# tusen-ai/simpledet

Measured on AMD Instinct MI355X. Metric: images/sec at 800x1333 FPN 512-RoI RoIAlign fwd+bwd, higher is better.
Workload: dtype f32; 1 GPU; fused FPN RoIAlign_v2 fwd+bwd, P2-P5 256ch 800x1333, N=2 img/GPU, 512 RoIs/img, 7x7x4 samples (BASELINE configs[1]); images_per_gpu=2, rois_per_image=512, argmax_state=packed u8 (decoded in backward)

## Files before the change

simpledet_amd/csrc/roi_align_common.h:

```cpp
#pragma once
#include "common.h"
#include "../../include/simpledet_ops.h"
#include <float.h>
#include <math.h>
#include <type_traits>
#include <hip/hip_fp16.h>

namespace sd {

struct RoiLevels {
  const float* data[SD_MAX_FPN_LEVELS];
  int H[SD_MAX_FPN_LEVELS], W[SD_MAX_FPN_LEVELS], stride[SD_MAX_FPN_LEVELS];
  float scale[SD_MAX_FPN_LEVELS];
  int nlvl;
  float canon_scale, canon_level, k_min, k_max;
};

__device__ __forceinline__ int fpn_level(float x1, float y1, float x2, float y2,
                                         const RoiLevels& L) {
  float area = (x2 - x1 + 1.f) * (y2 - y1 + 1.f);
  float s = sqrtf(area);
  float t = floorf(L.canon_level + log2f(s / L.canon_scale + 1e-6f));
  t = t < L.k_min ? L.k_min : (t > L.k_max ? L.k_max : t);
  if (!(t == t)) return -1;
// ... 162 lines not shown
constexpr int kBandHalo = 8;
constexpr int kBandMaxBands = 16;
constexpr int kBandNP = 4;
constexpr int kBandMaxUnits = 512;
constexpr int kBandFillCost = 140, kBandPlaneCost = 60, kBandSetupCost = 1500;
constexpr int kBandSub = 4;
constexpr int kBandFallbackWGs = 0;

typedef float v2f __attribute__((ext_vector_type(2)));

struct BandPlan {
  int owned[SD_MAX_FPN_LEVELS];
  int rows[SD_MAX_FPN_LEVELS];
  int nbands[SD_MAX_FPN_LEVELS];
  int g[SD_MAX_FPN_LEVELS];
  int unit_base[SD_MAX_FPN_LEVELS];
  int halo[SD_MAX_FPN_LEVELS];
  int nwg;
  int nunits;
  int grab;
  int gbias;
  int tail;
  int tail_planes;
  int pool;
  uint4* rowent;
  uint4* colent;
  float2* rowval;
  float2* colval;
  unsigned* items;
  int2* seg;
  unsigned char* fbflag;
  int* chan_ctr;
  int nlist, nent;
};

struct BandArgs {
  FwdArgs f;
  BandPlan p;
};

struct BwdArgs {
  RoiLevels L;
  const float* dy;
  const float* ax;
  const float* ay;
  const float* rois;
  float* dx;
  int B, C, R, PP, H, W;
  float scale;
  int filter_lvl;
  int band_rows, nbands;
  int req;
  int ablate;
};

struct BwdFusedArgs {
  RoiLevels L;
  const float* dy;
  const float* ax;
  const float* ay;
  const unsigned char* amax8;
  const float* coords;
  const float* rois;
  float* dx[SD_MAX_FPN_LEVELS];
  int band_rows[SD_MAX_FPN_LEVELS], nbands[SD_MAX_FPN_LEVELS];
  int block_end[SD_MAX_FPN_LEVELS];
// ... 33 lines not shown
```

simpledet_amd/csrc/roi_align_fwd.hip:

```cpp
#include "roi_align_common.h"

namespace sd {

__global__ __launch_bounds__(256) void roi_align_fwd_naive(FwdArgs a) {
  const int PP = a.PH * a.PW;
  const long count = (long)a.B * a.R * a.C * PP;
  for (long index = (long)blockIdx.x * blockDim.x + threadIdx.x; index < count;
       index += (long)gridDim.x * blockDim.x) {
    int pw = (int)(index % a.PW);
    int ph = (int)((index / a.PW) % a.PH);
    int c = (int)((index / PP) % a.C);
    int n = (int)(index / PP / a.C);
    const float* r = a.rois + (long)n * 4;
    float x1 = r[0], y1 = r[1], x2 = r[2], y2 = r[3];
    int lvl = 0;
    if (a.L.nlvl > 1) lvl = fpn_level(x1, y1, x2, y2, a.L);
    FwdOut o{0.f, -1.f, -1.f, 255};
    if (lvl >= 0) {
      int H = a.L.H[lvl], W = a.L.W[lvl];
      const float* plane = a.L.data[lvl] + ((long)(n / a.R) * a.C + c) * H * W;
      o = roi_align_fwd_elem(plane, H, W, x1, y1, x2, y2, a.L.scale[lvl], ph, pw, a.PH, a.PW);
    }
    if (a.L.nlvl > 1) o.val = o.val + 0.0f;
    a.out[index] = o.val;
    if (a.amax8) {
      a.amax8[((long)n * a.C + c) * amax_stride(PP) + ph * a.PW + pw] = (unsigned char)o.code;
    } else {
      a.ax[index] = o.ax;
      a.ay[index] = o.ay;
    }
  }
}

// ... 373 lines not shown
  }
}

template <int PH, int PW, int NROI, bool PK>
__global__ __launch_bounds__(512) void roi_align_fwd_tiled(FwdArgs a) {
  __shared__ FwdSmem<PH, PW, NROI> s;
  fwd_tiled_body<PH, PW, NROI, PK>(a, s, blockIdx.x);
}

__device__ __forceinline__ int band_fill(const float* gsrc, int len, float* buf, int wave, int lane) {
  const int shift = (int)(((uintptr_t)gsrc >> 2) & 3);
  const float* a0 = gsrc - shift;
  const int n4 = (shift + len + 3) >> 2;
  const int first_full = shift ? 1 : 0;
  const int last_full = ((shift + len) >> 2);
  const float4* s4 = reinterpret_cast<const float4*>(a0);
  float4* d4 = reinterpret_cast<float4*>(buf);
  for (int w4 = wave * kWave; w4 < last_full; w4 += kBandWaves * kWave) {
    const int i = w4 + lane;
    if (i >= first_full && i < last_full) __builtin_amdgcn_global_load_lds(s4 + i, d4 + w4, 16, 0, 0);
  }
  if (wave == 0) {
    if (shift && lane < 4 && lane >= shift && lane < shift + len)
      __builtin_amdgcn_global_load_lds(a0 + lane, buf, 4, 0, 0);
    if (last_full < n4 && last_full >= first_full && (last_full > 0 || !shift)) {
      const int j = last_full * 4 + lane;
      if (lane < 4 && j < shift + len) __builtin_amdgcn_global_load_lds(a0 + j, buf + last_full * 4, 4, 0, 0);
    }
  }
  return shift;
}

template <int POOL, bool PK, bool HALF = false>
__global__ __launch_bounds__(kBandThreads) void roi_align_fwd_band(BandArgs A) {
  using TIn = typename std::conditional<HALF, __half, float>::type;
  constexpr int AL = HALF ? 8 : 4;
  const FwdArgs& a = A.f;
  const BandPlan& P = A.p;
  constexpr int QL = POOL, IPP = kWave / QL;
  constexpr int NP = (PK && !HALF) ? kBandNP : kBandNP - 1, CAP = NP * kBandWaves * IPP;
  constexpr int PPG = POOL * POOL, PPSG = amax_stride(PPG);
  extern __shared__ __attribute__((aligned(16))) float band_smem[];
  const int tid = threadIdx.x, lane = tid & (kWave - 1);
  const int wave = __builtin_amdgcn_readfirstlane(tid / kWave);

#ifdef SD_PROFILING
  const long long t_entry = __builtin_readcyclecounter();
#endif
  __shared__ int v_unit[kBandMaxUnits], v_first[kBandMaxUnits], v_items[kBandMaxUnits];
  __shared__ int v_cost[kBandMaxUnits], v_start[kBandMaxUnits + 1];
  __shared__ int2 s_grab[2];
  __shared__ int s_pick;
  const int wg = (int)blockIdx.x - kBandFallbackWGs, nwg = (int)gridDim.x - kBandFallbackWGs;
  const int rsub = (a.R + kBandSub - 1) / kBandSub;
  auto level_of = [&](int u) {
    int l = 0;
    for (int k = 0; k < a.L.nlvl; ++k)
      if (a.L.stride[k] >= 0 && u >= P.unit_base[k]) l = k;
    return l;
  };
  __shared__ int s_nvu;
  auto wave_incl_scan = [&](int v) {
#pragma unroll
    for (int o = 1; o < kWave; o <<= 1) {
      const int t = __shfl_up(v, o);
      if (lane >= o) v += t;
    }
// ... 430 lines not shown
    for (int n0 = wg / nsl; n0 < nroi && wg / nsl < nslots; n0 += nslots * kWave) {
      const int nl = n0 + lane * nslots;
      int myflag = nl < nroi ? P.fbflag[nl] : 0;
      if (fast_void && myflag == 2) myflag = 0;
      unsigned long long todo = __ballot(myflag != 0);
      while (todo) {
      const int src = __builtin_ctzll(todo);
      todo &= todo - 1;
      const int n = n0 + src * nslots;
      const int flag = __builtin_amdgcn_readlane(myflag, src);
      const float4 bx = *reinterpret_cast<const float4*>(a.rois + (long)n * 4);
      const int lvl = a.L.nlvl > 1 ? fpn_level(bx.x, bx.y, bx.z, bx.w, a.L) : 0;
      for (int e = tid; e < csl * PPG; e += kBandThreads) {
        const int c = slice * csl + e / PPG, g = e % PPG;
        FwdOut o{0.f, -1.f, -1.f, 255};
        if (lvl >= 0 && flag == 1) {
          const int H = a.L.H[lvl], W = a.L.W[lvl];
          o = roi_align_fwd_elem(reinterpret_cast<const TIn*>(a.L.data[lvl]) + ((long)(n / a.R) * a.C + c) * H * W,
                                 H, W, bx.x, bx.y, bx.z, bx.w, a.L.scale[lvl], g / POOL, g % POOL, POOL, POOL);
        }
        if (a.L.nlvl > 1) o.val = o.val + 0.0f;
        if constexpr (HALF) reinterpret_cast<__half*>(a.out)[((long)n * a.C + c) * PPG + g] = __float2half(o.val);
        else a.out[((long)n * a.C + c) * PPG + g] = o.val;
        if (PK) {
          a.amax8[((long)n * a.C + c) * PPSG + g] = (unsigned char)o.code;
        } else {
          a.ax[((long)n * a.C + c) * PPG + g] = o.ax;
          a.ay[((long)n * a.C + c) * PPG + g] = o.ay;
        }
      }
      }
    }
    }
#ifdef SD_PROFILING
  if (a.dbg && lane == 0) {
    long long* d = a.dbg + ((long)blockIdx.x * kBandWaves + wave) * 8;
    d[0] = t_setup; d[1] = t_wait; d[2] = t_comp; d[3] = dbg_count;
    d[4] = __builtin_readcyclecounter() - t_begin; d[5] = t_begin - t_entry; d[6] = dbg_units; d[7] = t_begin;
  }
#endif
}

__global__ __launch_bounds__(512) void roi_align_fwd_quad(BandArgs A) {
  extern __shared__ __attribute__((aligned(16))) float band_smem[];
  const FwdArgs& a = A.f;
  const BandPlan& P = A.p;
  constexpr int T = 512, POOL = 7, PPG = POOL * POOL, NW = T / kWave;
  const int tid = threadIdx.x, lane = tid & (kWave - 1);
  const int wave = __builtin_amdgcn_readfirstlane(tid / kWave);
  const int G = a.C / 4;
  const int c = 4 * ((G & 7) == 0 ? (int)(blockIdx.x & 7) * (G >> 3) + (int)(blockIdx.x >> 3) : (int)blockIdx.x);
  const int img = blockIdx.y;
  const int H = a.L.H[0], W = a.L.W[0], HW = H * W;
  float4* pl = reinterpret_cast<float4*>(band_smem);
  float* st = band_smem + 4 * (HW + 1) + wave * (4 * PPG);
  const float* src = reinterpret_cast<const float*>(a.L.data[0]) + ((long)img * a.C + c) * HW;
  if ((HW & 3) == 0) {
    for (int i4 = tid; i4 < (HW >> 2); i4 += T) {
      const float4 v0 = *reinterpret_cast<const float4*>(src + 4 * i4);
      const float4 v1 = *reinterpret_cast<const float4*>(src + (long)HW + 4 * i4);
      const float4 v2 = *reinterpret_cast<const float4*>(src + 2L * HW + 4 * i4);
      const float4 v3 = *reinterpret_cast<const float4*>(src + 3L * HW + 4 * i4);
      pl[4 * i4 + 0] = make_float4(v0.x, v1.x, v2.x, v3.x);
      pl[4 * i4 + 1] = make_float4(v0.y, v1.y, v2.y, v3.y);
      pl[4 * i4 + 2] = make_float4(v0.z, v1.z, v2.z, v3.z);
      pl[4 * i4 + 3] = make_float4(v0.w, v1.w, v2.w, v3.w);
// ... 188 lines not shown
      int nbn = H <= rb ? 1 : (H + (rb - halo) - 1) / (rb - halo);
      const int cap = kBandNP * kBandWaves * (kWave / POOL);
      const long est = (long)a.R * POOL / (nvalid_lv > 0 ? nvalid_lv : 1);
      const int by_items = (int)((est * 5 + 4L * cap - 1) / (4L * cap));
      if (by_items > nbn && a.amax8) nbn = by_items;
      if (nbn > H) nbn = H;
      if (nbn > kBandMaxBands) nbn = kBandMaxBands;
      int owned = (H + nbn - 1) / nbn;
      if (nbn > 1)
        for (int o = owned; o < owned + 4 && o + halo <= rb; ++o)
          if (((long)o * W) % 4 == 0) { owned = o; break; }
      if (owned + halo > rb) owned = rb - halo;
      nbn = (H + owned - 1) / owned;
      if (nbn > kBandMaxBands) { ok = false; break; }
      P.nbands[l] = nbn;
      P.halo[l] = halo;
      P.owned[l] = nbn == 1 ? H : owned;
      P.rows[l] = nbn == 1 ? H : (owned + halo < H ? owned + halo : H);
      const long bstride = a.half_io ? (((long)P.rows[l] * W + 14) >> 3) * 8 : (((long)P.rows[l] * W + 4 + 3) & ~3L);
      int g = 1;
      for (int c = 2; c <= 8 && c <= gmax; c *= 2)
        if (a.C % c == 0 && c * bstride <= kBandBufFloats) g = c;
      if (bstride > kBandBufFloats) { ok = false; break; }
      P.g[l] = g;
      P.unit_base[l] = units;
      units += a.B * P.nbands[l];
    }
    auto al16 = [](size_t x) { return (x + 15) & ~(size_t)15; };
    const size_t ent = al16((size_t)nroi * POOL * sizeof(uint4));
    const size_t valb = a.amax8 ? 0 : al16((size_t)nroi * POOL * sizeof(float2));
    const size_t itemb = al16((size_t)a.B * SD_MAX_FPN_LEVELS * kBandSub * ((a.R + kBandSub - 1) / kBandSub) *
                              POOL * sizeof(unsigned));
    const size_t segb = al16((size_t)units * kBandSub * sizeof(int2));
    const size_t need = 16 + 2 * ent + 2 * valb + itemb + segb + al16(nroi) + kBandMaxUnits * sizeof(int);
    int wg = 0;
    P.nunits = units;
    P.grab = 4;
    P.gbias = 0;
    P.tail = 0;
    P.tail_planes = 8;
    {
      const int np = (a.amax8 && !a.half_io) ? kBandNP : kBandNP - 1;
      const long cap_launch = (long)np * kBandWaves * (kWave / POOL);
      if (units + (long)nroi * POOL / cap_launch > kBandMaxUnits) ok = false;
    }
    wg = kNumCU;
    if (ok && need <= workspace_bytes) {
      char* w = reinterpret_cast<char*>(((uintptr_t)workspace + 15) & ~(uintptr_t)15);
      P.rowent = reinterpret_cast<uint4*>(w); w += ent;
      P.colent = reinterpret_cast<uint4*>(w); w += ent;
      if (valb) {
        P.rowval = reinterpret_cast<float2*>(w); w += valb;
        P.colval = reinterpret_cast<float2*>(w); w += valb;
      }
      P.items = reinterpret_cast<unsigned*>(w); w += itemb;
      P.seg = reinterpret_cast<int2*>(w); w += segb;
      P.fbflag = reinterpret_cast<unsigned char*>(w); w += al16(nroi);
      P.chan_ctr = reinterpret_cast<int*>(w);
      P.nwg = wg;
      P.pool = POOL;
      A.f = a;
      const int nlist = a.B * a.L.nlvl * kBandSub, nent = cdiv((long)nroi * 2 * POOL, kBandThreads);
      const int ncoord = a.amax8 ? cdiv((long)nroi * 6 * POOL, kBandThreads) : 0;
      P.nlist = nlist; P.nent = nent;
      const int smem = 2 * kBandBufFloats * (int)sizeof(float);
      const bool merged = bplan && bplan->lists_units > 0 && bplan->PP == POOL * POOL;
      if (bplan_done) *bplan_done = merged;
      if (int e = launch_fwd_prep(A, POOL, nlist + nent + ncoord, merged ? bplan : nullptr, st)) return e;
      {
        const long HW0 = (long)a.L.H[0] * a.L.W[0];
        const size_t lds = (size_t)(HW0 + 1) * 16 + 8 * 4 * 49 * sizeof(float);
        if (!a.amax8 && !a.half_io && POOL == 7 && a.L.nlvl == 1 && a.L.stride[0] >= 0 && P.nbands[0] == 1 &&
            a.C % 4 == 0 && lds <= 78 * 1024 && a.B <= 65535 &&
            (((uintptr_t)a.L.data[0] | (uintptr_t)a.out | (uintptr_t)a.ax | (uintptr_t)a.ay) & 15) == 0 &&
            tuning("roi_align_fwd_quad", 1) == 1) {
          SD_HIP_CHECK(hipFuncSetAttribute((const void*)roi_align_fwd_quad, hipFuncAttributeMaxDynamicSharedMemorySize, (int)lds));
          hipLaunchKernelGGL(roi_align_fwd_quad, dim3(a.C / 4, a.B), dim3(512), lds, st, A);
          note_dispatch("sd::roi_fwd_prep_kernel<7> + sd::roi_align_fwd_quad");
          SD_LAUNCH_CHECK();
          return SD_OK;
        }
      }
#define SD_FWD_BAND(POOLV, PK)                                                                    \
  do {                                                                                            \
    auto k = roi_align_fwd_band<POOLV, PK>;                                                       \
    SD_HIP_CHECK(hipFuncSetAttribute((const void*)k, hipFuncAttributeMaxDynamicSharedMemorySize,  \
                                     smem));                                                      \
    hipLaunchKernelGGL(k, dim3(wg + kBandFallbackWGs), dim3(kBandThreads), smem, st, A);          \
  } while (0)
      if (a.half_io) {
#define SD_FWD_BAND_H(POOLV)                                                                      \
  do {                                                                                            \
    auto k = roi_align_fwd_band<POOLV, true, true>;                                               \
    SD_HIP_CHECK(hipFuncSetAttribute((const void*)k, hipFuncAttributeMaxDynamicSharedMemorySize,  \
                                     smem));                                                      \
    hipLaunchKernelGGL(k, dim3(wg + kBandFallbackWGs), dim3(kBandThreads), smem, st, A);          \
  } while (0)
        if (POOL == 7) SD_FWD_BAND_H(7); else SD_FWD_BAND_H(14);
#undef SD_FWD_BAND_H
      } else if (POOL == 7) {
        if (a.amax8) SD_FWD_BAND(7, true); else SD_FWD_BAND(7, false);
      } else {
        if (a.amax8) SD_FWD_BAND(14, true); else SD_FWD_BAND(14, false);
      }
#undef SD_FWD_BAND
      note_dispatch("sd::%s<%d> + sd::roi_align_fwd_band<%d,%s,%s>", merged ? "roi_prep_merged_kernel" : "roi_fwd_prep_kernel",
                    POOL, POOL, a.amax8 ? "true" : "false", a.half_io ? "true" : "false");
      SD_LAUNCH_CHECK();
      return SD_OK;
    }
  }
  if (a.half_io)
    return fail(SD_ERR_UNSUPPORTED, "fp16 RoIAlign runs on the band-resident kernel only: it needs the workspace, "
                "7x7 or 14x14 pooling, W in [2, 4095] and roi_align_fwd = 1, roi_align_fwd_band = 1");
  note_dispatch("sd::roi_align_fwd (tiled / naive fallback kernels: no workspace or a shape the band kernel does not take)");
  if (variant >= 1 && wide && a.PH == 7 && a.PW == 7) {
    if (a.amax8)
      hipLaunchKernelGGL((roi_align_fwd_tiled<7, 7, 4, true>), dim3(cdiv(nroi, 4) * a.nslice), dim3(512), 0, st, a);
    else
      hipLaunchKernelGGL((roi_align_fwd_tiled<7, 7, 4, false>), dim3(cdiv(nroi, 4) * a.nslice), dim3(512), 0, st, a);
  } else if (variant >= 1 && wide && a.PH == 14 && a.PW == 14) {
    if (a.amax8)
      hipLaunchKernelGGL((roi_align_fwd_tiled<14, 14, 1, true>), dim3(nroi * a.nslice), dim3(512), 0,
                         st, a);
    else
      hipLaunchKernelGGL((roi_align_fwd_tiled<14, 14, 1, false>), dim3(nroi * a.nslice), dim3(512),
                         0, st, a);
  } else {
    const int grid = (int)((count + 255) / 256 < 65536 * 16 ? (count + 255) / 256 : 65536 * 16);
    hipLaunchKernelGGL(roi_align_fwd_naive, dim3(grid), dim3(256), 0, st, a);
    if (a.amax8)
      hipLaunchKernelGGL(roi_coords_kernel, dim3(nroi), dim3(64), 0, st, a.rois, nroi, a.L, a.PH,
                         a.PW, a.coords);
  }
  SD_LAUNCH_CHECK();
  return SD_OK;
}

int check_dims(int B, int C, int R, int ph, int pw) {
  SD_REQUIRE(B >= 0 && C >= 0 && R >= 0, "negative dimension (B=%d C=%d R=%d)", B, C, R);
// ... 184 lines not shown
```

simpledet_amd/csrc/roi_align_lists.h:

```cpp
#pragma once
#include "roi_align_common.h"

namespace sd {

template <int PH, int PW, int THREADS>
__device__ __forceinline__ void bwd_band_list(const BwdFusedArgs& a, int lvl, int img, int nbands, int row0,
                                              int row1, float4 rb0, int* list, int* nlist, int* wcnt) {
  constexpr int NW = THREADS / kWave;
  const int tid = threadIdx.x, wave = tid / kWave, lane = tid & (kWave - 1);
  const int H = a.L.H[lvl];
  const float scale = a.L.scale[lvl];
  int base = 0, bound_sum = 0;
  for (int r0 = 0; r0 < a.R; r0 += THREADS) {
    const int r = r0 + tid;
    bool take = r < a.R && !(SD_ABLATE(a, 4));
    int weight = 0;
    if (take) {
      const float4 rb = r0 == 0 ? rb0 : *reinterpret_cast<const float4*>(a.rois + ((long)img * a.R + r) * 4);
      if (a.filter) take = fpn_level(rb.x, rb.y, rb.z, rb.w, a.L) == lvl;
      if (take && nbands > 1) {
        float s = fminr(fmaxr(rb.y * scale, 0.f), (float)(H - 1));
        float e = fminr(fmaxr(rb.w * scale, 0.f), (float)(H - 1));
        float lo = fminr(s, e) - 2.f, hi = fmaxr(s, e) + 2.f;
        if (hi < (float)row0 || lo > (float)(row1 - 1)) take = false;
      }
      if (take) {
        const float bwx = (rb.z - rb.x) * scale * (1.f / (float)PW), bwy = (rb.w - rb.y) * scale * (1.f / (float)PH);
        const float fx = 2.00002f * __builtin_amdgcn_rcpf(bwx), fy = 2.00002f * __builtin_amdgcn_rcpf(bwy);
        const int nx = (bwx > 0.f && fx < (float)PW) ? iminr((int)fx + 2, PW) : PW;
        const int ny = (bwy > 0.f && fy < (float)PH) ? iminr((int)fy + 2, PH) : PH;
        weight = nx * ny;
      }
    }
    const unsigned long long mask = __ballot(take);
    bound_sum += wave_sum_i32(weight);
    if (r0 > 0) __syncthreads();
    if (lane == 0) wcnt[wave] = __popcll(mask);
    __syncthreads();
    int off = base, total = 0;
#pragma unroll
    for (int w = 0; w < NW; ++w) {
      const int n = wcnt[w];
      if (w < wave) off += n;
      total += n;
    }
    if (take) list[off + __popcll(mask & ((1ull << lane) - 1))] = r;
    base += total;
  }
  if (lane == 0) atomicAdd(nlist + 1, bound_sum);
  if (tid == 0) nlist[0] = base;
  __syncthreads();
}

}
```

simpledet_amd/csrc/roi_align_prep.hip:

```cpp
#include "roi_align_lists.h"

namespace sd {

template <int POOL>
__device__ __forceinline__ void band_prep_block(const BandArgs& A, const int pblock, int nlist, int nent) {
  const FwdArgs& a = A.f;
  const BandPlan& P = A.p;
  const int tid = threadIdx.x, lane = tid & (kWave - 1);
  constexpr int LPR = POOL <= 8 ? 8 : 16;
  constexpr int RPP = kBandThreads / LPR;
  if (pblock < nlist) {
    __shared__ int hist[kBandMaxBands], cursor[kBandMaxBands];
    const int sub = pblock % kBandSub, lvl = (pblock / kBandSub) % a.L.nlvl;
    const int img = pblock / (kBandSub * a.L.nlvl);
    if (a.L.stride[lvl] < 0) return;
    int first_valid = 0;
    while (a.L.stride[first_valid] < 0) ++first_valid;
    const int H = a.L.H[lvl], W = a.L.W[lvl], nb = P.nbands[lvl], owned = P.owned[lvl];
    const float scale = a.L.scale[lvl];
    const int rsub = (a.R + kBandSub - 1) / kBandSub;
    const int rbeg = sub * rsub, rend = rbeg + rsub < a.R ? rbeg + rsub : a.R;
    if (tid < kBandMaxBands) hist[tid] = 0;
    __syncthreads();
    const int rr = tid / LPR, p = tid % LPR;
// ... 55 lines not shown
      int run = 0;
      for (int b = 0; b < nb; ++b) {
        cursor[b] = run;
        P.seg[(P.unit_base[lvl] + img * nb + b) * kBandSub + sub] = make_int2(run, hist[b]);
        run += hist[b];
      }
    }
    __syncthreads();
    auto emit = [&](int n, int band) {
      unsigned long long todo = __ballot(band >= 0);
      while (todo) {
        const int src = __builtin_ctzll(todo);
        const int bb = __builtin_amdgcn_readlane(band, src);
        const unsigned long long m = __ballot(band == bb);
        int base = 0;
        if (lane == src) base = atomicAdd(&cursor[bb], __popcll(m));
        base = __builtin_amdgcn_readlane(base, src);
        if (band == bb)
          items[base + __builtin_amdgcn_mbcnt_hi((unsigned)(m >> 32), __builtin_amdgcn_mbcnt_lo((unsigned)m, 0))] =
              (unsigned)n | ((unsigned)p << 16);
        todo &= ~m;
      }
    };
#pragma unroll
    for (int k = 0; k < KP; ++k)
      if (k < npass) emit(rbeg + k * RPP + rr, keep[k]);
    for (int k = KP; k < npass; ++k) {
      const int n = rbeg + k * RPP + rr;
      emit(n, classify(n));
    }
    return;
  }
  if (pblock == nlist && tid < kBandMaxUnits) P.chan_ctr[tid] = 0;
  const int eb = pblock - nlist;
  const int nroi = a.B * a.R;
  if (eb < nent) {
    const long e = (long)eb * kBandThreads + tid;
    if (e >= (long)nroi * 2 * POOL) return;
    const int p = (int)(e % POOL), ax = (int)((e / POOL) % 2), n = (int)(e / (2 * POOL));
    const float4 bx = *reinterpret_cast<const float4*>(a.rois + (long)n * 4);
    const int lvl = a.L.nlvl > 1 ? fpn_level(bx.x, bx.y, bx.z, bx.w, a.L) : 0;
    if (lvl < 0) return;
    const int H = a.L.H[lvl], W = a.L.W[lvl];
    float val[2] = {0.f, 0.f}, frac[2] = {0.f, 0.f};
    int off[4];
    const int cnt = ax == 0 ? axis_samples(p, POOL, bx.y, bx.w, a.L.scale[lvl], H, W, val, frac, off)
                            : axis_samples(p, POOL, bx.x, bx.z, a.L.scale[lvl], W, 1, val, frac, off);
    const float qnan = __int_as_float(0x7fc00000);
    const bool v0 = cnt >= 1, v1 = cnt >= 2;
    uint4 en;
    if (ax == 0) {
      en.x = (v0 ? (unsigned)off[0] | (off[1] != off[0] ? 1u << 20 : 0u) : 0u) | (cnt < 0 ? 1u << 31 : 0u);
      en.y = v1 ? (unsigned)off[2] | (off[3] != off[2] ? 1u << 20 : 0u) : 0u;
    } else {
      en.x = (v0 ? (unsigned)off[0] | (off[1] == off[0] ? 1u << 12 : 0u) : 0u) |
             (v1 ? (unsigned)off[2] << 13 | (off[3] == off[2] ? 1u << 25 : 0u) : 0u) | (cnt < 0 ? 1u << 26 : 0u);
      en.y = 0u;
    }
    en.z = __float_as_uint(v0 ? frac[0] : qnan);
    en.w = __float_as_uint(v1 ? frac[1] : qnan);
    (ax == 0 ? P.rowent : P.colent)[(long)n * POOL + p] = en;
    if (P.rowval) (ax == 0 ? P.rowval : P.colval)[(long)n * POOL + p] = make_float2(val[0], val[1]);
    return;
  }
  if (a.amax8) {
    const long e = (long)(eb - nent) * kBandThreads + tid;
    if (e >= (long)nroi * 6 * POOL) return;
    const int j = (int)(e % (6 * POOL)), n = (int)(e / (6 * POOL));
    const float4 bx = *reinterpret_cast<const float4*>(a.rois + (long)n * 4);
    const int lvl = a.L.nlvl > 1 ? fpn_level(bx.x, bx.y, bx.z, bx.w, a.L) : 0;
    if (lvl < 0) return;
    const bool row = j < 3 * POOL;
    const int jj = row ? j : j - 3 * POOL;
    const float v = row ? sample_coord(jj / 3, POOL, bx.y, bx.w, a.L.scale[lvl], a.L.H[lvl], jj % 3)
                        : sample_coord(jj / 3, POOL, bx.x, bx.z, a.L.scale[lvl], a.L.W[lvl], jj % 3);
    float* cb = a.coords + (long)n * kCoordWords * (POOL + POOL);
    cb[j] = v;
    store_tap(cb + 3 * (POOL + POOL) + 2 * j, v, row ? a.L.H[lvl] : a.L.W[lvl]);
  }
}

template <int POOL>
__global__ __launch_bounds__(kBandThreads) void roi_fwd_prep_kernel(BandArgs A) {
  band_prep_block<POOL>(A, (int)blockIdx.x, A.p.nlist, A.p.nent);
}

template <int PH, int PW, int THREADS, int PARTS>
__device__ __forceinline__ void bwd_lists_block(const BwdFusedArgs& a, int block, float* smem) {
  int* list = reinterpret_cast<int*>(smem);
  int* nlist = list + a.R;
  const int tid = threadIdx.x;
  const int NP = PARTS + (a.pix_bound_words > 0 ? 1 : 0);
  const int unit = block / NP, part = block % NP;
  int li = 0;
  while (li + 1 < a.nlaunch && unit >= a.unit_base[li + 1]) ++li;
  const int lvl = a.order[li];
  const int u = unit - a.unit_base[li];
  const int nbands = a.nbands[lvl];
  const int img = u / nbands, band = u % nbands;
  const int row0 = band * a.band_rows[lvl];
  const int row1 = iminr(row0 + a.band_rows[lvl], a.L.H[lvl]);
  float4 rb0 = make_float4(0.f, 0.f, 0.f, 0.f);
  if (tid < a.R) rb0 = *reinterpret_cast<const float4*>(a.rois + ((long)img * a.R + tid) * 4);
  if (tid < 8) nlist[tid] = 0;
  __syncthreads();
  bwd_band_list<PH, PW, THREADS>(a, lvl, img, nbands, row0, row1, rb0, list, nlist, nlist + 8);
  int* dst = a.ws_list + (long)unit * (a.R + 2);
  const int nl = nlist[0];
  const int H = a.L.H[lvl], W = a.L.W[lvl];
  constexpr int CS = 2;
  const int DW = ((W - 1) >> CS) + 2, DH = ((row1 - row0 - 1) >> CS) + 2;
  const bool pix = DW * DH <= a.pix_bound_words;
  if (part == 0) {
    if (tid == 0) dst[0] = nl;
    if (tid == 1 && !pix) dst[1] = nlist[1];
    for (int i = tid; i < nl; i += THREADS) dst[2 + i] = list[i];
  }
  if (part == PARTS && !pix) return;
  if (part == PARTS) {
    constexpr int NW = THREADS / kWave;
    const int wave = tid / kWave, lane = tid & (kWave - 1);
    int* D = nlist + 8 + 16;
    for (int i = tid; i < DW * DH; i += THREADS) D[i] = 0;
    __syncthreads();
    const float scale = a.L.scale[lvl];
    for (int j = tid; j < nl; j += THREADS) {
      const float4 rb = *reinterpret_cast<const float4*>(a.rois + ((long)img * a.R + list[j]) * 4);
      const float xs = fminr(fmaxr(rb.x * scale, 0.f), (float)(W - 1)), xe = fminr(fmaxr(rb.z * scale, 0.f), (float)(W - 1));
      const float ys = fminr(fmaxr(rb.y * scale, 0.f), (float)(H - 1)), ye = fminr(fmaxr(rb.w * scale, 0.f), (float)(H - 1));
      const float xlo = fminr(xs, xe) - 2.f, xhi = fmaxr(xs, xe) + 2.f;
      const float ylo = fminr(ys, ye) - 2.f, yhi = fmaxr(ys, ye) + 2.f;
      int x0 = 0, x1 = W - 1, y0 = 0, y1 = H - 1;
      if (xlo >= -2.f && xhi <= (float)(W + 1)) { x0 = imaxr((int)floorf(xlo), 0); x1 = iminr((int)ceilf(xhi), W - 1); }
      if (ylo >= -2.f && yhi <= (float)(H + 1)) { y0 = imaxr((int)floorf(ylo), 0); y1 = iminr((int)ceilf(yhi), H - 1); }
      y0 = imaxr(y0, row0) - row0;
      y1 = iminr(y1, row1 - 1) - row0;
      if (y0 > y1) continue;
      x0 >>= CS; x1 >>= CS; y0 >>= CS; y1 >>= CS;
      const float bwx = (rb.z - rb.x) * scale * (1.f / (float)PW), bwy = (rb.w - rb.y) * scale * (1.f / (float)PH);
      const float fx = 2.00002f * __builtin_amdgcn_rcpf(bwx), fy = 2.00002f * __builtin_amdgcn_rcpf(bwy);
      const int nx = (bwx > 0.f && fx < (float)PW) ? iminr((int)fx + 2, PW) : PW;
      const int ny = (bwy > 0.f && fy < (float)PH) ? iminr((int)fy + 2, PH) : PH;
      const int w = nx * ny;
      atomicAdd(D + y0 * DW + x0, w);
      atomicAdd(D + y0 * DW + x1 + 1, -w);
      atomicAdd(D + (y1 + 1) * DW + x0, -w);
      atomicAdd(D + (y1 + 1) * DW + x1 + 1, w);
    }
    __syncthreads();
    for (int y = wave; y < DH; y += NW) {
      int carry = 0;
      for (int xb = 0; xb < DW; xb += kWave) {
        const int x = xb + lane;
        const int v = wave_scan_i32(x < DW ? D[y * DW + x] : 0) + carry;
        if (x < DW) D[y * DW + x] = v;
        carry = __builtin_amdgcn_readlane(v, kWave - 1);
      }
    }
    __syncthreads();
    int m = 0;
    for (int x = tid; x < DW; x += THREADS) {
      int run = 0;
      for (int y = 0; y < DH; ++y) {
        run += D[y * DW + x];
        m = imaxr(m, run);
      }
    }
    if (m > 0) atomicMax(nlist + 5, m);
    __syncthreads();
    if (tid == 0) dst[1] = iminr(nlist[1], nlist[5]);
    return;
  }
  if (a.ws_taps) {
    constexpr int NE = 3 * (PH + PW), TS = kTapMainWords * (PH + PW), SS = kTapSideWords * (PH + PW);
    const int H = a.L.H[lvl], W = a.L.W[lvl];
    const float scale = a.L.scale[lvl];
    float* tdst = a.ws_taps + (long)unit * a.R * (2 * NE);
    float* sdst = tdst + (long)a.R * TS;
    for (int i = part * THREADS + tid; i < nl * NE; i += PARTS * THREADS) {
      const int j = i / NE, e = i - j * NE;
      const bool row = e < 3 * PH;
      const int ee = row ? e : e - 3 * PH;
      const float4 bx = *reinterpret_cast<const float4*>(a.rois + ((long)img * a.R + list[j]) * 4);
      const float v = row ? sample_coord(ee / 3, PH, bx.y, bx.w, scale, H, ee % 3)
                          : sample_coord(ee / 3, PW, bx.x, bx.z, scale, W, ee % 3);
      const int size = row ? H : W;
      const int lo = iminr(imaxr((int)floorf(v), 0), size - 1);
      const int hi = iminr(imaxr((int)ceilf(v), 0), size - 1);
      const float frac = (lo == hi) ? 0.5f : (v - (float)lo);
      unsigned w0 = (unsigned)(4 * lo) | ((unsigned)(4 * hi) << 16);
      if (row) {
        const unsigned o0 = (lo >= row0 && lo < row1) ? (unsigned)(4 * (lo - row0) * W) : 0xffffu;
        const unsigned o1 = (hi >= row0 && hi < row1) ? (unsigned)(4 * (hi - row0) * W) : 0xffffu;
        w0 = o0 | (o1 << 16);
      }
      const int bin = (row ? 0 : PH) + ee / 3, cand = ee % 3;
      float* dstp = cand < 2 ? tdst + (long)j * TS + 2 * (2 * bin + cand) : sdst + (long)j * SS + 2 * bin;
      *reinterpret_cast<float2*>(dstp) = make_float2(__uint_as_float(w0), frac);
    }
  }
}

template <int PH, int PW>
__global__ __launch_bounds__(512) void roi_align_bwd_lists(BwdFusedArgs a) {
  extern __shared__ __attribute__((aligned(16))) float smem[];
  bwd_lists_block<PH, PW, 512, kListSplit>(a, (int)blockIdx.x, smem);
}

template <int POOL>
__global__ __launch_bounds__(kBandThreads) void roi_prep_merged_kernel(BandArgs A, BwdFusedArgs b, int nfwd) {
  extern __shared__ __attribute__((aligned(16))) float smem[];
  if ((int)blockIdx.x < nfwd) band_prep_block<POOL>(A, (int)blockIdx.x, A.p.nlist, A.p.nent);
  else bwd_lists_block<POOL, POOL, kBandThreads, kMergedListSplit>(b, (int)blockIdx.x - nfwd, smem);
}


int launch_fwd_prep(const BandArgs& A, int pool, int nblocks, const BwdFusedArgs* bplan, hipStream_t st) {
  const FwdArgs& a = A.f;
  if (bplan) {
    const dim3 g((unsigned)(nblocks + bplan->lists_units * (kMergedListSplit + (bplan->pix_bound_words > 0 ? 1 : 0))));
    const size_t lds = (size_t)(a.R + 8 + 16 + bplan->pix_bound_words) * 4;
    if (pool == 7) hipLaunchKernelGGL((roi_prep_merged_kernel<7>), g, dim3(kBandThreads), lds, st, A, *bplan, nblocks);
    else hipLaunchKernelGGL((roi_prep_merged_kernel<14>), g, dim3(kBandThreads), lds, st, A, *bplan, nblocks);
  } else {
    if (pool == 7) hipLaunchKernelGGL((roi_fwd_prep_kernel<7>), dim3(nblocks), dim3(kBandThreads), 0, st, A);
    else hipLaunchKernelGGL((roi_fwd_prep_kernel<14>), dim3(nblocks), dim3(kBandThreads), 0, st, A);
  }
  SD_LAUNCH_CHECK();
  return SD_OK;
}

int launch_bwd_lists(const BwdFusedArgs& a, int units, hipStream_t st) {
  const size_t lds = (size_t)(a.R + 8 + 16 + a.pix_bound_words) * 4;
// ... 9 lines not shown
```

simpledet_amd/csrc/runtime.hip:

```cpp
#include "common.h"
#include <stdarg.h>
#include "../../include/simpledet_ops.h"
#include <atomic>
#include <string.h>
#include <hip/hip_fp16.h>

namespace sd {

char* err_buf() {
  static thread_local char buf[512] = {0};
  return buf;
}

int fail(int code, const char* fmt, ...) {
  va_list ap;
  va_start(ap, fmt);
  vsnprintf(err_buf(), 512, fmt, ap);
  va_end(ap);
  return code;
}

namespace {
struct Knob {
  const char* key;
  std::atomic<int> value;
  std::atomic<bool> set;
  Knob(const char* k, int v, bool s) : key(k), value(v), set(s) {}
};
Knob g_knobs[] = {
    {"roi_align_fwd", 0, false},
    {"roi_align_fwd_band", 0, false},
    {"roi_align_fwd_quad", 0, false},
    {"roi_align_bwd", 0, false},
    {"roi_align_bwd_flt4", 0, false},
    {"roi_align_bwd_fx", 0, false},
    {"roi_align_bwd_pixbound", 0, false},
    {"roi_align_bwd_lists", 0, false},
    {"roi_pool_fwd", 0, false},
    {"roi_pool_bwd", 0, false},
    {"deform_psroi_bwd_patch", 0, false},
    {"proposal_topk", 0, false},
    {"soft_nms_threads", 0, false},
    {"deform_gemm_split", 0, false},
    {"deform_gemm_vecstore", 0, false},
    {"deform_gemm_nt", 0, false},
    {"deform_gemm_ksplit", 0, false},
    {"dcn_im2col", 0, false},
    {"dcn_window", 0, false},
    {"dcn_im2col_pipe", 0, false},
    {"dcn_col2im", 0, false},
    {"dcn_col2im_fx", 0, false},
    {"dcn_coord", 0, false},
    {"dcn_fused", 0, false},
    {"dcn_fused_tile", 0, false},
#ifdef SD_PROFILING
    {"roi_align_fwd_ablate", 0, false},
    {"roi_pool_fwd_ablate", 0, false},
    {"roi_align_bwd_ablate", 0, false},
    {"roi_align_dbg_lo", 0, false},
    {"roi_align_dbg_hi", 0, false},
    {"gemm_ablate", 0, false},
    {"gemm_dbg_cap", 0, false},
    {"dcn_im2col_nt", 0, false},
    {"dcn_fused_ablate", 0, false},
#endif
// ... 120 lines not shown
```

Baseline: 10700 images/s.

## Run coordinate-table and backward-plan tasks as a ticketed tail inside forward band kernel

Moves the coordinate-table blocks and the backward list/tap planning blocks out of the prep kernel. They now run as tail work in the forward band kernel: workgroups that finish band work grab tasks through an atomic ticket counter. This is meant to fill idle CUs during the band kernel's ragged end and to shorten the serial prep kernel. In exchange it adds an atomic and barriers per task, an extra kernel argument, and reads RoiLevels through the kernarg pointer, which depends on argument layout.

```diff
diff --git a/simpledet_amd/csrc/roi_align_common.h b/simpledet_amd/csrc/roi_align_common.h
--- a/simpledet_amd/csrc/roi_align_common.h
+++ b/simpledet_amd/csrc/roi_align_common.h
@@ -218,6 +218,8 @@
   unsigned char* fbflag;
   int* chan_ctr;
   int nlist, nent;
+  int* ticket;
+  int tail_coord, tail_lists;
 };
 
 struct BandArgs {
diff --git a/simpledet_amd/csrc/roi_align_fwd.hip b/simpledet_amd/csrc/roi_align_fwd.hip
--- a/simpledet_amd/csrc/roi_align_fwd.hip
+++ b/simpledet_amd/csrc/roi_align_fwd.hip
@@ -1,4 +1,4 @@
-#include "roi_align_common.h"
+#include "roi_align_lists.h"
 
 namespace sd {
 
@@ -438,7 +438,7 @@
 }
 
 template <int POOL, bool PK, bool HALF = false>
-__global__ __launch_bounds__(kBandThreads) void roi_align_fwd_band(BandArgs A) {
+__global__ __launch_bounds__(kBandThreads) void roi_align_fwd_band(BandArgs A, BwdFusedArgs bplan) {
   using TIn = typename std::conditional<HALF, __half, float>::type;
   constexpr int AL = HALF ? 8 : 4;
   const FwdArgs& a = A.f;
@@ -935,6 +935,23 @@
       }
     }
     }
+  if (P.ticket) {
+    const int ntasks = P.tail_coord + P.tail_lists;
+    asm volatile("s_waitcnt vmcnt(0)" ::: "memory");
+    static_assert(offsetof(BandArgs, f) == 0 && offsetof(FwdArgs, L) == 0, "RoiLevels leads the kernel arguments");
+    const RoiLevels* geom_p = (const RoiLevels*)__builtin_amdgcn_kernarg_segment_ptr();
+    asm volatile("" : "+s"(geom_p));
+    const RoiLevels& geom = *geom_p;
+    for (;;) {
+      __syncthreads();
+      if (tid == 0) s_pick = __hip_atomic_fetch_add(P.ticket, 1, __ATOMIC_RELAXED, __HIP_MEMORY_SCOPE_AGENT);
+      __syncthreads();
+      const int t = s_pick;
+      if (t >= ntasks) break;
+      if (PK && t < P.tail_coord) coords_block<POOL>(a, geom, t);
+      else bwd_lists_block<POOL, POOL, kBandThreads, kMergedListSplit>(bplan, t - P.tail_coord, band_smem);
+    }
+  }
 #ifdef SD_PROFILING
   if (a.dbg && lane == 0) {
     long long* d = a.dbg + ((long)blockIdx.x * kBandWaves + wave) * 8;
@@ -1189,7 +1206,7 @@
     const size_t itemb = al16((size_t)a.B * SD_MAX_FPN_LEVELS * kBandSub * ((a.R + kBandSub - 1) / kBandSub) *
                               POOL * sizeof(unsigned));
     const size_t segb = al16((size_t)units * kBandSub * sizeof(int2));
-    const size_t need = 16 + 2 * ent + 2 * valb + itemb + segb + al16(nroi) + kBandMaxUnits * sizeof(int);
+    const size_t need = 16 + 2 * ent + 2 * valb + itemb + segb + al16(nroi) + kBandMaxUnits * sizeof(int) + 16;
     int wg = 0;
     P.nunits = units;
     P.grab = 4;
@@ -1223,7 +1240,19 @@
       const int smem = 2 * kBandBufFloats * (int)sizeof(float);
       const bool merged = bplan && bplan->lists_units > 0 && bplan->PP == POOL * POOL;
       if (bplan_done) *bplan_done = merged;
-      if (int e = launch_fwd_prep(A, POOL, nlist + nent + ncoord, merged ? bplan : nullptr, st)) return e;
+      const int nbwd = merged ? bplan->lists_units * (kMergedListSplit + (bplan->pix_bound_words > 0 ? 1 : 0)) : 0;
+      const size_t tail_lds = merged ? (size_t)(a.R + 8 + 16 + bplan->pix_bound_words) * 4 : 0;
+      const bool tail = tuning("roi_align_plan_tail", 1) == 1 && ncoord + nbwd > 0 && tail_lds <= (size_t)smem;
+      static const BwdFusedArgs no_plan{};
+      const BwdFusedArgs& tplan = tail && merged ? *bplan : no_plan;
+      if (tail) {
+        P.ticket = P.chan_ctr + kBandMaxUnits;
+        P.tail_coord = ncoord;
+        P.tail_lists = nbwd;
+      }
+      if (int e = tail ? launch_fwd_prep(A, POOL, nlist + nent, nullptr, st)
+                       : launch_fwd_prep(A, POOL, nlist + nent + ncoord, merged ? bplan : nullptr, st))
+        return e;
       {
         const long HW0 = (long)a.L.H[0] * a.L.W[0];
         const size_t lds = (size_t)(HW0 + 1) * 16 + 8 * 4 * 49 * sizeof(float);
@@ -1243,7 +1272,7 @@
     auto k = roi_align_fwd_band<POOLV, PK>;                                                       \
     SD_HIP_CHECK(hipFuncSetAttribute((const void*)k, hipFuncAttributeMaxDynamicSharedMemorySize,  \
                                      smem));                                                      \
-    hipLaunchKernelGGL(k, dim3(wg + kBandFallbackWGs), dim3(kBandThreads), smem, st, A);          \
+    hipLaunchKernelGGL(k, dim3(wg + kBandFallbackWGs), dim3(kBandThreads), smem, st, A, tplan);   \
   } while (0)
       if (a.half_io) {
 #define SD_FWD_BAND_H(POOLV)                                                                      \
@@ -1251,7 +1280,7 @@
     auto k = roi_align_fwd_band<POOLV, true, true>;                                               \
     SD_HIP_CHECK(hipFuncSetAttribute((const void*)k, hipFuncAttributeMaxDynamicSharedMemorySize,  \
                                      smem));                                                      \
-    hipLaunchKernelGGL(k, dim3(wg + kBandFallbackWGs), dim3(kBandThreads), smem, st, A);          \
+    hipLaunchKernelGGL(k, dim3(wg + kBandFallbackWGs), dim3(kBandThreads), smem, st, A, tplan);   \
   } while (0)
         if (POOL == 7) SD_FWD_BAND_H(7); else SD_FWD_BAND_H(14);
 #undef SD_FWD_BAND_H
@@ -1261,8 +1290,10 @@
         if (a.amax8) SD_FWD_BAND(14, true); else SD_FWD_BAND(14, false);
       }
 #undef SD_FWD_BAND
-      note_dispatch("sd::%s<%d> + sd::roi_align_fwd_band<%d,%s,%s>", merged ? "roi_prep_merged_kernel" : "roi_fwd_prep_kernel",
-                    POOL, POOL, a.amax8 ? "true" : "false", a.half_io ? "true" : "false");
+      char tail_note[96] = "";
+      if (tail) snprintf(tail_note, sizeof(tail_note), " (tail tasks: %d coordinate table + %d backward plan)", ncoord, nbwd);
+      note_dispatch("sd::%s<%d> + sd::roi_align_fwd_band<%d,%s,%s>%s", merged && !tail ? "roi_prep_merged_kernel" : "roi_fwd_prep_kernel",
+                    POOL, POOL, a.amax8 ? "true" : "false", a.half_io ? "true" : "false", tail_note);
       SD_LAUNCH_CHECK();
       return SD_OK;
     }
diff --git a/simpledet_amd/csrc/roi_align_lists.h b/simpledet_amd/csrc/roi_align_lists.h
--- a/simpledet_amd/csrc/roi_align_lists.h
+++ b/simpledet_amd/csrc/roi_align_lists.h
@@ -16,7 +16,8 @@
     bool take = r < a.R && !(SD_ABLATE(a, 4));
     int weight = 0;
     if (take) {
-      const float4 rb = r0 == 0 ? rb0 : *reinterpret_cast<const float4*>(a.rois + ((long)img * a.R + r) * 4);
+      float4 rb = rb0;
+      if (r0 != 0) rb = *reinterpret_cast<const float4*>(a.rois + ((long)img * a.R + r) * 4);
       if (a.filter) take = fpn_level(rb.x, rb.y, rb.z, rb.w, a.L) == lvl;
       if (take && nbands > 1) {
         float s = fminr(fmaxr(rb.y * scale, 0.f), (float)(H - 1));
@@ -52,4 +53,138 @@
   __syncthreads();
 }
 
+template <int POOL>
+__device__ __forceinline__ void coords_block(const FwdArgs& a, const RoiLevels& G, int cb) {
+  const long e = (long)cb * kBandThreads + threadIdx.x;
+  if (e >= (long)a.B * a.R * 6 * POOL) return;
+  const int j = (int)(e % (6 * POOL)), n = (int)(e / (6 * POOL));
+  const float4 bx = *reinterpret_cast<const float4*>(a.rois + (long)n * 4);
+  const int lvl = a.L.nlvl > 1 ? fpn_level(bx.x, bx.y, bx.z, bx.w, a.L) : 0;
+  if (lvl < 0) return;
+  const float scale = G.scale[lvl];
+  const int H = G.H[lvl], W = G.W[lvl];
+  const bool row = j < 3 * POOL;
+  const int jj = row ? j : j - 3 * POOL;
+  const float v = row ? sample_coord(jj / 3, POOL, bx.y, bx.w, scale, H, jj % 3)
+                      : sample_coord(jj / 3, POOL, bx.x, bx.z, scale, W, jj % 3);
+  float* cbase = a.coords + (long)n * kCoordWords * (POOL + POOL);
+  cbase[j] = v;
+  store_tap(cbase + 3 * (POOL + POOL) + 2 * j, v, row ? H : W);
 }
+
+template <int PH, int PW, int THREADS, int PARTS>
+__device__ __forceinline__ void bwd_lists_block(const BwdFusedArgs& a, int block, float* smem) {
+  int* list = reinterpret_cast<int*>(smem);
+  int* nlist = list + a.R;
+  const int tid = threadIdx.x;
+  const int NP = PARTS + (a.pix_bound_words > 0 ? 1 : 0);
+  const int unit = block / NP, part = block % NP;
+  int li = 0;
+  while (li + 1 < a.nlaunch && unit >= a.unit_base[li + 1]) ++li;
+  const int lvl = a.order[li];
+  const int u = unit - a.unit_base[li];
+  const int nbands = a.nbands[lvl];
+  const int img = u / nbands, band = u % nbands;
+  const int row0 = band * a.band_rows[lvl];
+  const int row1 = iminr(row0 + a.band_rows[lvl], a.L.H[lvl]);
+  float4 rb0 = make_float4(0.f, 0.f, 0.f, 0.f);
+  if (tid < a.R) rb0 = *reinterpret_cast<const float4*>(a.rois + ((long)img * a.R + tid) * 4);
+  if (tid < 8) nlist[tid] = 0;
+  __syncthreads();
+  bwd_band_list<PH, PW, THREADS>(a, lvl, img, nbands, row0, row1, rb0, list, nlist, nlist + 8);
+  int* dst = a.ws_list + (long)unit * (a.R + 2);
+  const int nl = nlist[0];
+  const int H = a.L.H[lvl], W = a.L.W[lvl];
+  constexpr int CS = 2;
+  const int DW = ((W - 1) >> CS) + 2, DH = ((row1 - row0 - 1) >> CS) + 2;
+  const bool pix = DW * DH <= a.pix_bound_words;
+  if (part == 0) {
+    if (tid == 0) dst[0] = nl;
+    if (tid == 1 && !pix) dst[1] = nlist[1];
+    for (int i = tid; i < nl; i += THREADS) dst[2 + i] = list[i];
+  }
+  if (part == PARTS && !pix) return;
+  if (part == PARTS) {
+    constexpr int NW = THREADS / kWave;
+    const int wave = tid / kWave, lane = tid & (kWave - 1);
+    int* D = nlist + 8 + 16;
+    for (int i = tid; i < DW * DH; i += THREADS) D[i] = 0;
+    __syncthreads();
+    const float scale = a.L.scale[lvl];
+    for (int j = tid; j < nl; j += THREADS) {
+      const float4 rb = *reinterpret_cast<const float4*>(a.rois + ((long)img * a.R + list[j]) * 4);
+      const float xs = fminr(fmaxr(rb.x * scale, 0.f), (float)(W - 1)), xe = fminr(fmaxr(rb.z * scale, 0.f), (float)(W - 1));
+      const float ys = fminr(fmaxr(rb.y * scale, 0.f), (float)(H - 1)), ye = fminr(fmaxr(rb.w * scale, 0.f), (float)(H - 1));
+      const float xlo = fminr(xs, xe) - 2.f, xhi = fmaxr(xs, xe) + 2.f;
+      const float ylo = fminr(ys, ye) - 2.f, yhi = fmaxr(ys, ye) + 2.f;
+      int x0 = 0, x1 = W - 1, y0 = 0, y1 = H - 1;
+      if (xlo >= -2.f && xhi <= (float)(W + 1)) { x0 = imaxr((int)floorf(xlo), 0); x1 = iminr((int)ceilf(xhi), W - 1); }
+      if (ylo >= -2.f && yhi <= (float)(H + 1)) { y0 = imaxr((int)floorf(ylo), 0); y1 = iminr((int)ceilf(yhi), H - 1); }
+      y0 = imaxr(y0, row0) - row0;
+      y1 = iminr(y1, row1 - 1) - row0;
+      if (y0 > y1) continue;
+      x0 >>= CS; x1 >>= CS; y0 >>= CS; y1 >>= CS;
+      const float bwx = (rb.z - rb.x) * scale * (1.f / (float)PW), bwy = (rb.w - rb.y) * scale * (1.f / (float)PH);
+      const float fx = 2.00002f * __builtin_amdgcn_rcpf(bwx), fy = 2.00002f * __builtin_amdgcn_rcpf(bwy);
+      const int nx = (bwx > 0.f && fx < (float)PW) ? iminr((int)fx + 2, PW) : PW;
+      const int ny = (bwy > 0.f && fy < (float)PH) ? iminr((int)fy + 2, PH) : PH;
+      const int w = nx * ny;
+      atomicAdd(D + y0 * DW + x0, w);
+      atomicAdd(D + y0 * DW + x1 + 1, -w);
+      atomicAdd(D + (y1 + 1) * DW + x0, -w);
+      atomicAdd(D + (y1 + 1) * DW + x1 + 1, w);
+    }
+    __syncthreads();
+    for (int y = wave; y < DH; y += NW) {
+      int carry = 0;
+      for (int xb = 0; xb < DW; xb += kWave) {
+        const int x = xb + lane;
+        const int v = wave_scan_i32(x < DW ? D[y * DW + x] : 0) + carry;
+        if (x < DW) D[y * DW + x] = v;
+        carry = __builtin_amdgcn_readlane(v, kWave - 1);
+      }
+    }
+    __syncthreads();
+    int m = 0;
+    for (int x = tid; x < DW; x += THREADS) {
+      int run = 0;
+      for (int y = 0; y < DH; ++y) {
+        run += D[y * DW + x];
+        m = imaxr(m, run);
+      }
+    }
+    if (m > 0) atomicMax(nlist + 5, m);
+    __syncthreads();
+    if (tid == 0) dst[1] = iminr(nlist[1], nlist[5]);
+    return;
+  }
+  if (a.ws_taps) {
+    constexpr int NE = 3 * (PH + PW), TS = kTapMainWords * (PH + PW), SS = kTapSideWords * (PH + PW);
+    const float scale = a.L.scale[lvl];
+    float* tdst = a.ws_taps + (long)unit * a.R * (2 * NE);
+    float* sdst = tdst + (long)a.R * TS;
+    for (int i = part * THREADS + tid; i < nl * NE; i += PARTS * THREADS) {
+      const int j = i / NE, e = i - j * NE;
+      const bool row = e < 3 * PH;
+      const int ee = row ? e : e - 3 * PH;
+      const float4 bx = *reinterpret_cast<const float4*>(a.rois + ((long)img * a.R + list[j]) * 4);
+      const float v = row ? sample_coord(ee / 3, PH, bx.y, bx.w, scale, H, ee % 3)
+                          : sample_coord(ee / 3, PW, bx.x, bx.z, scale, W, ee % 3);
+      const int size = row ? H : W;
+      const int lo = iminr(imaxr((int)floorf(v), 0), size - 1);
+      const int hi = iminr(imaxr((int)ceilf(v), 0), size - 1);
+      const float frac = (lo == hi) ? 0.5f : (v - (float)lo);
+      unsigned w0 = (unsigned)(4 * lo) | ((unsigned)(4 * hi) << 16);
+      if (row) {
+        const unsigned o0 = (lo >= row0 && lo < row1) ? (unsigned)(4 * (lo - row0) * W) : 0xffffu;
+        const unsigned o1 = (hi >= row0 && hi < row1) ? (unsigned)(4 * (hi - row0) * W) : 0xffffu;
+        w0 = o0 | (o1 << 16);
+      }
+      const int bin = (row ? 0 : PH) + ee / 3, cand = ee % 3;
+      float* dstp = cand < 2 ? tdst + (long)j * TS + 2 * (2 * bin + cand) : sdst + (long)j * SS + 2 * bin;
+      *reinterpret_cast<float2*>(dstp) = make_float2(__uint_as_float(w0), frac);
+    }
+  }
+}
+
+}
diff --git a/simpledet_amd/csrc/roi_align_prep.hip b/simpledet_amd/csrc/roi_align_prep.hip
--- a/simpledet_amd/csrc/roi_align_prep.hip
+++ b/simpledet_amd/csrc/roi_align_prep.hip
@@ -111,6 +111,7 @@
     return;
   }
   if (pblock == nlist && tid < kBandMaxUnits) P.chan_ctr[tid] = 0;
+  if (pblock == nlist && tid == 0 && P.ticket) *P.ticket = 0;
   const int eb = pblock - nlist;
   const int nroi = a.B * a.R;
   if (eb < nent) {
@@ -142,142 +143,12 @@
     if (P.rowval) (ax == 0 ? P.rowval : P.colval)[(long)n * POOL + p] = make_float2(val[0], val[1]);
     return;
   }
-  if (a.amax8) {
-    const long e = (long)(eb - nent) * kBandThreads + tid;
-    if (e >= (long)nroi * 6 * POOL) return;
-    const int j = (int)(e % (6 * POOL)), n = (int)(e / (6 * POOL));
-    const float4 bx = *reinterpret_cast<const float4*>(a.rois + (long)n * 4);
-    const int lvl = a.L.nlvl > 1 ? fpn_level(bx.x, bx.y, bx.z, bx.w, a.L) : 0;
-    if (lvl < 0) return;
-    const bool row = j < 3 * POOL;
-    const int jj = row ? j : j - 3 * POOL;
-    const float v = row ? sample_coord(jj / 3, POOL, bx.y, bx.w, a.L.scale[lvl], a.L.H[lvl], jj % 3)
-                        : sample_coord(jj / 3, POOL, bx.x, bx.z, a.L.scale[lvl], a.L.W[lvl], jj % 3);
-    float* cb = a.coords + (long)n * kCoordWords * (POOL + POOL);
-    cb[j] = v;
-    store_tap(cb + 3 * (POOL + POOL) + 2 * j, v, row ? a.L.H[lvl] : a.L.W[lvl]);
-  }
+  if (a.amax8) coords_block<POOL>(a, a.L, eb - nent);
 }
 
 template <int POOL>
 __global__ __launch_bounds__(kBandThreads) void roi_fwd_prep_kernel(BandArgs A) {
   band_prep_block<POOL>(A, (int)blockIdx.x, A.p.nlist, A.p.nent);
-}
-
-template <int PH, int PW, int THREADS, int PARTS>
-__device__ __forceinline__ void bwd_lists_block(const BwdFusedArgs& a, int block, float* smem) {
-  int* list = reinterpret_cast<int*>(smem);
-  int* nlist = list + a.R;
-  const int tid = threadIdx.x;
-  const int NP = PARTS + (a.pix_bound_words > 0 ? 1 : 0);
-  const int unit = block / NP, part = block % NP;
-  int li = 0;
-  while (li + 1 < a.nlaunch && unit >= a.unit_base[li + 1]) ++li;
-  const int lvl = a.order[li];
-  const int u = unit - a.unit_base[li];
-  const int nbands = a.nbands[lvl];
-  const int img = u / nbands, band = u % nbands;
-  const int row0 = band * a.band_rows[lvl];
-  const int row1 = iminr(row0 + a.band_rows[lvl], a.L.H[lvl]);
-  float4 rb0 = make_float4(0.f, 0.f, 0.f, 0.f);
-  if (tid < a.R) rb0 = *reinterpret_cast<const float4*>(a.rois + ((long)img * a.R + tid) * 4);
-  if (tid < 8) nlist[tid] = 0;
-  __syncthreads();
-  bwd_band_list<PH, PW, THREADS>(a, lvl, img, nbands, row0, row1, rb0, list, nlist, nlist + 8);
-  int* dst = a.ws_list + (long)unit * (a.R + 2);
-  const int nl = nlist[0];
-  const int H = a.L.H[lvl], W = a.L.W[lvl];
-  constexpr int CS = 2;
-  const int DW = ((W - 1) >> CS) + 2, DH = ((row1 - row0 - 1) >> CS) + 2;
-  const bool pix = DW * DH <= a.pix_bound_words;
-  if (part == 0) {
-    if (tid == 0) dst[0] = nl;
-    if (tid == 1 && !pix) dst[1] = nlist[1];
-    for (int i = tid; i < nl; i += THREADS) dst[2 + i] = list[i];
-  }
-  if (part == PARTS && !pix) return;
-  if (part == PARTS) {
-    constexpr int NW = THREADS / kWave;
-    const int wave = tid / kWave, lane = tid & (kWave - 1);
-    int* D = nlist + 8 + 16;
-    for (int i = tid; i < DW * DH; i += THREADS) D[i] = 0;
-    __syncthreads();
-    const float scale = a.L.scale[lvl];
-    for (int j = tid; j < nl; j += THREADS) {
-      const float4 rb = *reinterpret_cast<const float4*>(a.rois + ((long)img * a.R + list[j]) * 4);
-      const float xs = fminr(fmaxr(rb.x * scale, 0.f), (float)(W - 1)), xe = fminr(fmaxr(rb.z * scale, 0.f), (float)(W - 1));
-      const float ys = fminr(fmaxr(rb.y * scale, 0.f), (float)(H - 1)), ye = fminr(fmaxr(rb.w * scale, 0.f), (float)(H - 1));
-      const float xlo = fminr(xs, xe) - 2.f, xhi = fmaxr(xs, xe) + 2.f;
-      const float ylo = fminr(ys, ye) - 2.f, yhi = fmaxr(ys, ye) + 2.f;
-      int x0 = 0, x1 = W - 1, y0 = 0, y1 = H - 1;
-      if (xlo >= -2.f && xhi <= (float)(W + 1)) { x0 = imaxr((int)floorf(xlo), 0); x1 = iminr((int)ceilf(xhi), W - 1); }
-      if (ylo >= -2.f && yhi <= (float)(H + 1)) { y0 = imaxr((int)floorf(ylo), 0); y1 = iminr((int)ceilf(yhi), H - 1); }
-      y0 = imaxr(y0, row0) - row0;
-      y1 = iminr(y1, row1 - 1) - row0;
-      if (y0 > y1) continue;
-      x0 >>= CS; x1 >>= CS; y0 >>= CS; y1 >>= CS;
-      const float bwx = (rb.z - rb.x) * scale * (1.f / (float)PW), bwy = (rb.w - rb.y) * scale * (1.f / (float)PH);
-      const float fx = 2.00002f * __builtin_amdgcn_rcpf(bwx), fy = 2.00002f * __builtin_amdgcn_rcpf(bwy);
-      const int nx = (bwx > 0.f && fx < (float)PW) ? iminr((int)fx + 2, PW) : PW;
-      const int ny = (bwy > 0.f && fy < (float)PH) ? iminr((int)fy + 2, PH) : PH;
-      const int w = nx * ny;
-      atomicAdd(D + y0 * DW + x0, w);
-      atomicAdd(D + y0 * DW + x1 + 1, -w);
-      atomicAdd(D + (y1 + 1) * DW + x0, -w);
-      atomicAdd(D + (y1 + 1) * DW + x1 + 1, w);
-    }
-    __syncthreads();
-    for (int y = wave; y < DH; y += NW) {
-      int carry = 0;
-      for (int xb = 0; xb < DW; xb += kWave) {
-        const int x = xb + lane;
-        const int v = wave_scan_i32(x < DW ? D[y * DW + x] : 0) + carry;
-        if (x < DW) D[y * DW + x] = v;
-        carry = __builtin_amdgcn_readlane(v, kWave - 1);
-      }
-    }
-    __syncthreads();
-    int m = 0;
-    for (int x = tid; x < DW; x += THREADS) {
-      int run = 0;
-      for (int y = 0; y < DH; ++y) {
-        run += D[y * DW + x];
-        m = imaxr(m, run);
-      }
-    }
-    if (m > 0) atomicMax(nlist + 5, m);
-    __syncthreads();
-    if (tid == 0) dst[1] = iminr(nlist[1], nlist[5]);
-    return;
-  }
-  if (a.ws_taps) {
-    constexpr int NE = 3 * (PH + PW), TS = kTapMainWords * (PH + PW), SS = kTapSideWords * (PH + PW);
-    const int H = a.L.H[lvl], W = a.L.W[lvl];
-    const float scale = a.L.scale[lvl];
-    float* tdst = a.ws_taps + (long)unit * a.R * (2 * NE);
-    float* sdst = tdst + (long)a.R * TS;
-    for (int i = part * THREADS + tid; i < nl * NE; i += PARTS * THREADS) {
-      const int j = i / NE, e = i - j * NE;
-      const bool row = e < 3 * PH;
-      const int ee = row ? e : e - 3 * PH;
-      const float4 bx = *reinterpret_cast<const float4*>(a.rois + ((long)img * a.R + list[j]) * 4);
-      const float v = row ? sample_coord(ee / 3, PH, bx.y, bx.w, scale, H, ee % 3)
-                          : sample_coord(ee / 3, PW, bx.x, bx.z, scale, W, ee % 3);
-      const int size = row ? H : W;
-      const int lo = iminr(imaxr((int)floorf(v), 0), size - 1);
-      const int hi = iminr(imaxr((int)ceilf(v), 0), size - 1);
-      const float frac = (lo == hi) ? 0.5f : (v - (float)lo);
-      unsigned w0 = (unsigned)(4 * lo) | ((unsigned)(4 * hi) << 16);
-      if (row) {
-        const unsigned o0 = (lo >= row0 && lo < row1) ? (unsigned)(4 * (lo - row0) * W) : 0xffffu;
-        const unsigned o1 = (hi >= row0 && hi < row1) ? (unsigned)(4 * (hi - row0) * W) : 0xffffu;
-        w0 = o0 | (o1 << 16);
-      }
-      const int bin = (row ? 0 : PH) + ee / 3, cand = ee % 3;
-      float* dstp = cand < 2 ? tdst + (long)j * TS + 2 * (2 * bin + cand) : sdst + (long)j * SS + 2 * bin;
-      *reinterpret_cast<float2*>(dstp) = make_float2(__uint_as_float(w0), frac);
-    }
-  }
 }
 
 template <int PH, int PW>
diff --git a/simpledet_amd/csrc/runtime.hip b/simpledet_amd/csrc/runtime.hip
--- a/simpledet_amd/csrc/runtime.hip
+++ b/simpledet_amd/csrc/runtime.hip
@@ -31,6 +31,7 @@
     {"roi_align_fwd", 0, false},
     {"roi_align_fwd_band", 0, false},
     {"roi_align_fwd_quad", 0, false},
+    {"roi_align_plan_tail", 0, false},
     {"roi_align_bwd", 0, false},
     {"roi_align_bwd_flt4", 0, false},
     {"roi_align_bwd_fx", 0, false},
```

Result: faster. 10940 images/s (median of 6 runs) (+2.3%).
